# algbio/founderblockgraphs

Hardware: AMD Instinct MI355X
Metric: MSA columns segmented/sec (higher is better)
Workload: dtype u32

## Files before the change

### founderblockgraphs_amd/csrc/fbg_internal.h

```cpp
#pragma once
#include <cstring>
#include <cstdlib>
#include <hip/hip_runtime.h>
#include <stdint.h>
#include <string>
#include "../../include/fbg_hip.h"

#define FBG_WAVE 64

struct DevBuf {
    void *p = nullptr;
    size_t cap = 0;
    template <class T> T *as() const { return reinterpret_cast<T *>(p); }
};

struct Stager {
    void *base = nullptr;
    size_t slot_bytes = 0;
    int nslots = 0;
    hipEvent_t *ev = nullptr;
    hipStream_t stream = nullptr;
};

struct StageTimer {
// ... 72 lines not shown
    DevBuf gbits;
    DevBuf gwin_rows;
    const uint64_t *grs_ebits = nullptr;
    bool grs_flagged = false;
    bool pairs_similar = false;
    bool grs_ties_done = false;
    bool gpart = false;
    bool grs_part_failed = false;
    uint32_t grs_t = 1;
    uint64_t grs_redone = 0;
    bool spanned = false;
    DevBuf sp_cells;
    DevBuf sp_flagT;
    bool sp_key_flags = false;
    uint64_t alloc_calls = 0, alloc_us = 0;
    int sp_decline = 0;
    bool sp_key_flags_sorted = false;
    DevBuf sp_cwin;
    DevBuf sp_tiles, sp_gstart, sp_gcol, sp_gflags, sp_rstart, sp_rid, sp_gplo, sp_gphi, sp_gval, sp_odd, sp_irr, sp_chain, sp_slow, sp_mins;
    uint32_t sp_chain_n = 0, sp_slow_n = 0;
    uint64_t sp_G = 0, sp_R = 0, sp_n_irr = 0, sp_work = 0;
    uint32_t sp_n_odd[4] = {0, 0, 0, 0}, sp_odd_cap = 0;
    const uint32_t *sort_payload = nullptr;
    int64_t msd_decline = -1;
    int dp_kind = -1;
    bool cells_built = false;
    uint8_t ignore_tab[256] = {0};
    uint64_t *rk_keys = nullptr;
    int rk_b = 0, rk_key_bits = 0, rk_K = 0;
    int rk_layout = 0, rk_pb = 0;
    bool part_active = false;
    int part = 0, nparts = 1;
    uint64_t part_count = 0;
    uint64_t part_T = 0;
    uint32_t part_gmin = 0;

    DevBuf keysA, keysB, valsA, valsB, grp, flags, list, tie_list, big_groups, tmp, small, scalars;
    DevBuf msd_ext;
    DevBuf kargs;
    alignas(16) unsigned char kargs_host[512];
    DevBuf msd_w, msd_v;
    DevBuf dp_a, dp_b, dp_c, dp_d, dp_e, dp_f, dp_g, dp_h, io_a, io_b, io_c, io_d;
    DevBuf bt_up, bt_dep;
    DevBuf ps_a, ps_b, ps_c, ps_d, ps_e, ps_f, ps_g, ps_h;

    StageTimer timers[FBG_STAGE_COUNT];
};

int fbg_fail(fbg_ctx *ctx, int code, const char *fmt, ...);
#define FBG_HIP_TRY(ctx, expr)                                                              \
    do {                                                                                    \
        hipError_t e_ = (expr);                                                             \
        if (e_ != hipSuccess)                                                               \
            return fbg_fail((ctx), e_ == hipErrorOutOfMemory ? FBG_ERR_OOM : FBG_ERR_HIP,   \
                            "%s failed: %s (%s:%d)", #expr, hipGetErrorString(e_), __FILE__, \
                            __LINE__);                                                      \
    } while (0)
#define FBG_TRY(expr)                \
    do {                             \
        int rc_ = (expr);            \
        if (rc_ != FBG_OK) return rc_; \
    } while (0)

int fbg_reserve(fbg_ctx *ctx, DevBuf &b, size_t bytes);
int fbg_upload(fbg_ctx *ctx, void *d_dst, const void *h_src, size_t bytes);
int fbg_download(fbg_ctx *ctx, void *h_dst, const void *d_src, size_t bytes);
void fbg_release(fbg_ctx *ctx, DevBuf &b);
// ... 77 lines not shown
```

### founderblockgraphs_amd/csrc/rank_common.h

```cpp
#pragma once
#include "fbg_internal.h"
#include "text_cmp.h"

#define RS_TG 4

__device__ __forceinline__ uint32_t rs_key_lcp(uint64_t a, uint64_t c, int b, int key_bits)
{
    const uint64_t d = a ^ c;
    const uint32_t bits = (uint32_t)(__clzll((long long)d) - (64 - key_bits));
    const uint32_t inv_b = (65536u + (uint32_t)b - 1) / (uint32_t)b;
    return (bits * inv_b) >> 16;
}

struct RankArgs {
    uint32_t magic32;
    uint64_t magic64;
    uint64_t *keys;
    uint32_t *vals;
    uint64_t pmask;
    int pb;
    const uint8_t *T;
    uint64_t N, n;
    uint64_t Ntext;
    uint64_t own_lo, own_hi;
    int first_part, last_part;
    int part_mode;
    int values_only;
    uint32_t row_len;
    uint32_t g_min;
    int b, key_bits, K, reversed;
    uint32_t *gmax;
    uint32_t *cand;
    uint32_t *blk_count;
    uint32_t region;
    uint32_t *ties;
    uint32_t *tie_count;
    uint32_t tie_region;
    uint2 *pairs;
    int pair_codes;
    unsigned long long *pair_stats;
    uint32_t *pair_count;
    uint32_t *pm;
    uint32_t *big;
    unsigned long long *counters;
};

struct Slot {
    uint64_t key;
    uint64_t pos;
    uint32_t col;
    uint32_t rem;
};

__device__ __forceinline__ uint32_t rs_col_of_rem(const RankArgs &a, uint32_t rem)
{
    return rem == 0 ? (uint32_t)a.n : (a.reversed ? rem - 1 : (uint32_t)a.n - rem);
}
template <int L> struct PosT { typedef uint32_t type; };
template <> struct PosT<FBG_SLOTS_WIDE> { typedef uint64_t type; };
template <int L> __device__ __forceinline__ uint64_t rs_key(const RankArgs &a, uint64_t k) { return a.keys[k] >> a.pb; }
template <int L> __device__ __forceinline__ uint64_t rs_pos_of(const RankArgs &a, uint64_t w, uint32_t v)
{
    if (L == FBG_SLOTS_PACKED) return w & a.pmask;
    if (L == FBG_SLOTS_WIDE) return ((w & a.pmask) << 32) | v;
    return v;
}
template <int L> __device__ __forceinline__ uint64_t rs_pos(const RankArgs &a, uint64_t k)
{
    return rs_pos_of<L>(a, L == FBG_SLOTS_PAIRS ? 0ull : a.keys[k], L == FBG_SLOTS_PACKED ? 0u : a.vals[k]);
}
template <int L> __device__ __forceinline__ void rs_set_pos(const RankArgs &a, uint64_t k, uint64_t p)
{
    if (L == FBG_SLOTS_PACKED) a.keys[k] = (a.keys[k] & ~a.pmask) | p;
    else if (L == FBG_SLOTS_WIDE) { a.keys[k] = (a.keys[k] & ~a.pmask) | (p >> 32); a.vals[k] = (uint32_t)p; }
    else a.vals[k] = (uint32_t)p;
// ... 139 lines not shown
        uint32_t mr = 0;
        for (;;) {
            const uint32_t rj = v.rem(j);
            mr = max(mr, rj);
            run = run || rj == rem;
            cnt++;
            if (j + 1 >= hi_i || v.key(j + 1) != kn) break;
            if (cnt == RS_TG) { run = true; break; }
            j++;
        }
        mrn = mr;
    }
    if (edge || run) { want_cand = true; return; }
    const uint32_t lp = has_prev ? min(min(rs_key_lcp(kp, key, a.b, a.key_bits), rem), mrp) : 0u;
    const uint32_t ln = has_next ? min(min(rs_key_lcp(key, kn, a.b, a.key_bits), rem), mrn) : 0u;
    const uint32_t g = max(lp, ln) + 1;
    if (g >= a.g_min || rem <= 64) rs_update(a, rs_col_of_rem(a, rem), g);
}


static inline int rs_layout(const KeyGeom &g) { return g.packed ? FBG_SLOTS_PACKED : g.wide ? FBG_SLOTS_WIDE : FBG_SLOTS_PAIRS; }

static inline void rs_args_init(fbg_ctx *ctx, RankArgs &a, uint64_t *keys, uint32_t *vals, uint64_t slots, int layout, int pb, int b,
                         int key_bits, int K)
{
    a.keys = keys; a.vals = vals; a.T = ctx->text.as<uint8_t>();
    a.pb = layout != FBG_SLOTS_PAIRS ? pb : 0; a.pmask = layout != FBG_SLOTS_PAIRS ? (1ull << pb) - 1 : 0;
    a.N = slots; a.Ntext = ctx->N; a.n = ctx->n; a.row_len = (uint32_t)(ctx->n + 1);
    a.own_lo = 0; a.own_hi = slots; a.first_part = a.last_part = 1; a.part_mode = 0; a.values_only = 0;
    a.magic32 = (uint32_t)((1ull << 32) / (ctx->n + 1));
    a.magic64 = ~0ull / (ctx->n + 1);
    a.b = b; a.key_bits = key_bits; a.K = K; a.reversed = ctx->reversed;
    a.gmax = ctx->gmax.as<uint32_t>();
    a.cand = nullptr; a.pm = nullptr; a.blk_count = nullptr; a.region = 0;
    a.ties = nullptr; a.tie_count = nullptr; a.tie_region = 0; a.pairs = nullptr; a.pair_count = nullptr; a.pair_codes = 0;
    a.pair_stats = nullptr;
    a.big = ctx->big_groups.as<uint32_t>();
    a.counters = ctx->scalars.as<unsigned long long>() + 32;
    a.g_min = 0;
}

static inline void rs_remember(fbg_ctx *ctx, uint64_t *keys, uint32_t *vals, const KeyGeom &g)
{
    ctx->rk_keys = keys; ctx->sa_ptr = vals;
    ctx->rk_layout = rs_layout(g); ctx->rk_pb = g.pb;
    ctx->rk_b = g.b; ctx->rk_key_bits = g.key_bits; ctx->rk_K = g.K;
}
```

### founderblockgraphs_amd/csrc/rank_scan.hip

```cpp
#include <algorithm>
#include <cstring>
#include <vector>
#include "fbg_internal.h"
#include "text_cmp.h"
#include <rocprim/rocprim.hpp>

#include "rank_common.h"

#define RS_ITEMS 4
#define RS_THREADS 256
#define RS_CHUNK (RS_THREADS * RS_ITEMS)

template <int L, bool PLAIN> __global__ __launch_bounds__(RS_THREADS) __attribute__((amdgpu_waves_per_eu(7, 8))) void k_rank_scan(RankArgs a)
{
    __shared__ uint64_t skey[RS_CHUNK + 2 * RS_HALO];
    __shared__ uint32_t srem[RS_CHUNK + 2 * RS_HALO];
    __shared__ uint16_t sq[RS_CHUNK];
    __shared__ uint32_t sqn, s_cand_n, s_tie_n;
    const int lane = threadIdx.x & 63;
    const uint64_t nchunks = (a.own_hi - a.own_lo + RS_CHUNK - 1) / RS_CHUNK;
    if (threadIdx.x == 0) { s_cand_n = 0; s_tie_n = 0; }
    uint64_t w[RS_ITEMS + 1];
    uint32_t v[RS_ITEMS + 1];
    const int my_i = RS_HALO + RS_ITEMS * (int)threadIdx.x;
    const int halo_i = (int)threadIdx.x < RS_HALO ? (int)threadIdx.x : RS_CHUNK + (int)threadIdx.x;
    auto fetch = [&](uint64_t c) {
        const uint64_t base = a.own_lo + c * RS_CHUNK;
        const int lo_i = c == 0 ? RS_HALO : 0;
        const int hi_i = (int)min((uint64_t)(RS_CHUNK + 2 * RS_HALO), a.own_hi - base + RS_HALO);
#pragma unroll
        for (int r = 0; r < RS_ITEMS; r++) {
            w[r] = 0; v[r] = 0;
            if (my_i + r < hi_i) {
                w[r] = a.keys[base + (uint64_t)(my_i + r - RS_HALO)];
                if (L != FBG_SLOTS_PACKED) v[r] = a.vals[base + (uint64_t)(my_i + r - RS_HALO)];
            }
        }
        w[RS_ITEMS] = 0; v[RS_ITEMS] = 0;
// ... 407 lines not shown
            const uint32_t ln = k + 1 < N ? rs_key_lcp(key, kn, b, key_bits) : 0u;
            bin = min(max(lp, ln) + 1, 63u);
        }
    }
    {
        const int lane = threadIdx.x & 63;
        unsigned long long rest = __ballot(bin != 0xffffffffu);
        while (rest) {
            const int l = __ffsll((long long)rest) - 1;
            const uint32_t v = __shfl(bin, l, 64);
            const unsigned long long same = __ballot(bin == v);
            if (lane == l) { if (v == 64) atomicAdd(&sties, (uint32_t)__popcll(same)); else atomicAdd(&sh[v], (uint32_t)__popcll(same)); }
            rest &= ~same;
        }
    }
    __syncthreads();
    if (threadIdx.x < 64 && sh[threadIdx.x]) atomicAdd(&hist[threadIdx.x], sh[threadIdx.x]);
    if (threadIdx.x == 0) {
        atomicAdd(&counters[2], (unsigned long long)sties);
        atomicAdd(&counters[3], (unsigned long long)min((uint64_t)256, N - (uint64_t)blockIdx.x * 1024 * 256));
    }
}

__global__ void k_count_unfilled(const uint32_t *__restrict__ gmax, uint64_t n, uint32_t g_min, int reversed,
                                 unsigned long long *__restrict__ counters)
{
    const uint64_t x = (uint64_t)blockIdx.x * blockDim.x + threadIdx.x;
    const uint64_t rem = reversed ? x + 1 : n - x;
    const bool miss = x < n && rem > 64 && gmax[x] < g_min;
    const unsigned long long mask = __ballot(miss);
    if ((threadIdx.x & 63) == 0 && mask) atomicAdd(&counters[1 + 3], (unsigned long long)__popcll(mask));
}

__global__ void k_cand_compact(const uint32_t *__restrict__ regions, const uint32_t *__restrict__ counts,
                               const uint32_t *__restrict__ offsets, uint32_t region, uint32_t *__restrict__ out)
{
    const uint32_t c = counts[blockIdx.x] < region ? counts[blockIdx.x] : region, o = offsets[blockIdx.x];
    for (uint32_t i = threadIdx.x; i < c; i += blockDim.x) out[o + i] = regions[(size_t)blockIdx.x * region + i];
}

#define RS_BIG_GROUPS 1024
#define RS_BIG_MEMBERS 8192
template <int L> __global__ void k_tie_groups(RankArgs a, uint64_t T, int by_list)
{
    const uint64_t t = (uint64_t)blockIdx.x * blockDim.x + threadIdx.x;
    if (t >= T) return;
    const uint64_t k0 = by_list ? (uint64_t)a.cand[t] : a.own_lo + t;
    const uint64_t key = rs_key<L>(a, k0);
    if (k0 > a.own_lo && rs_key<L>(a, k0 - 1) == key) return;
    if (k0 + 1 >= a.own_hi || rs_key<L>(a, k0 + 1) != key) return;
    uint32_t s = 1;
    while (k0 + s < a.own_hi && s <= RS_BIG_MEMBERS && rs_key<L>(a, k0 + s) == key) s++;
    if (s > 64) {
        if (s > RS_BIG_MEMBERS) { a.counters[1] = 1; return; }
        const unsigned long long e = atomicAdd(&a.counters[5], 1ull);
        if (e >= RS_BIG_GROUPS) { a.counters[1] = 1; return; }
        a.big[2 * e] = (uint32_t)k0;
        a.big[2 * e + 1] = s;
        return;
    }
    typedef typename PosT<L>::type pos_t;
    pos_t pos[64];
    uint32_t from = (uint32_t)a.K;
    for (uint32_t i = 0; i < s; i++) {
        pos[i] = (pos_t)rs_pos<L>(a, k0 + i);
        if (rs_rem<L>(a, pos[i]) < (uint32_t)a.K) from = 0;
    }
    for (uint32_t i = 1; i < s; i++) {
        const pos_t cur = pos[i];
        uint32_t j = i;
        while (j > 0) {
            const pos_t o = pos[j - 1];
            const uint32_t h = fbg_extend_match(a.T, (uint64_t)o + from, (uint64_t)cur + from, 0);
            if (a.T[(uint64_t)o + from + h] < a.T[(uint64_t)cur + from + h]) break;
            pos[j] = o;
            j--;
        }
        pos[j] = cur;
    }
    for (uint32_t i = 0; i < s; i++) rs_set_pos<L>(a, k0 + i, pos[i]);
}

template <int L> __global__ __launch_bounds__(256) void k_tie_big(RankArgs a, int exact)
{
    __shared__ uint32_t pos_lo[RS_BIG_MEMBERS];
    __shared__ uint8_t pos_hi[L == FBG_SLOTS_WIDE ? RS_BIG_MEMBERS : 1];
    __shared__ uint8_t cls[RS_BIG_MEMBERS];
    __shared__ uint32_t offs[66];
    __shared__ uint32_t q_start, q_count;
    if (blockIdx.x >= a.counters[5]) return;
    const uint64_t k0 = a.big[2 * blockIdx.x];
    const uint32_t s = a.big[2 * blockIdx.x + 1];
    auto member = [&](uint32_t i) -> uint64_t {
        return L == FBG_SLOTS_WIDE ? ((uint64_t)pos_hi[L == FBG_SLOTS_WIDE ? i : 0] << 32) | pos_lo[i] : (uint64_t)pos_lo[i];
    };
    if (threadIdx.x < 66) offs[threadIdx.x] = 0;
    __syncthreads();
    for (uint32_t i = threadIdx.x; i < s; i += blockDim.x) {
        const uint64_t p = rs_pos<L>(a, k0 + i);
        const uint32_t c = min(rs_rem<L>(a, p), (uint32_t)a.K);
        pos_lo[i] = (uint32_t)p;
        if (L == FBG_SLOTS_WIDE) pos_hi[L == FBG_SLOTS_WIDE ? i : 0] = (uint8_t)(p >> 32);
        cls[i] = (uint8_t)c;
        atomicAdd(&offs[c + 1], 1u);
    }
    __syncthreads();
    if (threadIdx.x == 0) {
        q_count = offs[a.K + 1];
        for (int c = 1; c <= a.K + 1; c++) offs[c] += offs[c - 1];
        q_start = offs[a.K];
    }
    __syncthreads();
    if (!exact) {
// ... 25 lines not shown
    for (uint32_t i = threadIdx.x; i < s; i += blockDim.x) {
        const uint64_t p = member(i);
        uint32_t rank = 0;
        for (uint32_t j = 0; j < s; j++) {
            if (j == i) continue;
            const uint64_t o = member(j);
            const uint32_t h = fbg_extend_match(a.T, o, p, 0);
            rank += a.T[o + h] < a.T[p + h] ? 1u : 0u;
        }
        rs_set_pos<L>(a, k0 + rank, p);
    }
}

template <int L> __device__ __forceinline__ uint32_t rs_slot_lcp(const RankArgs &a, uint64_t k)
{
    if (k == (a.first_part ? a.own_lo : 0) || k >= (a.last_part ? a.own_hi : a.N)) return 0;
    const Slot x = rs_slot<L>(a, k - 1), y = rs_slot<L>(a, k);
    if (x.key != y.key) return min(min(rs_key_lcp(x.key, y.key, a.b, a.key_bits), x.rem), y.rem);
    const uint32_t from = (x.rem < (uint32_t)a.K || y.rem < (uint32_t)a.K) ? 0u : (uint32_t)a.K;
    return fbg_clamp_lcp(fbg_extend_match(a.T, (uint64_t)x.pos + from, (uint64_t)y.pos + from, 0) + from);
}

template <int L> __global__ void k_rank_materialize(RankArgs a, uint32_t *sa, uint32_t *isa, uint32_t *pl, uint32_t *pr)
{
    const uint64_t k = (uint64_t)blockIdx.x * blockDim.x + threadIdx.x;
    if (k >= a.N) return;
    const uint32_t p = (uint32_t)rs_pos<L>(a, k);
    sa[k] = p;
    isa[p] = (uint32_t)k;
    pl[p] = rs_slot_lcp<L>(a, k);
    pr[p] = rs_slot_lcp<L>(a, k + 1);
}

template <int L> __global__ void k_runs(RankArgs a, uint64_t T)
{
    const uint64_t t = (uint64_t)blockIdx.x * blockDim.x + threadIdx.x;
    if (t >= T) return;
    const uint64_t k0 = a.cand[t];
    const uint32_t col = rs_col<L>(a, k0);
    if (col == a.n) return;
    if (k0 > a.own_lo && rs_col<L>(a, k0 - 1) == col) return;
    const uint64_t lo_slot = a.first_part ? a.own_lo : 0, hi_slot = a.last_part ? a.own_hi : a.N;
    uint64_t ks = k0;
    while (ks > lo_slot && rs_col<L>(a, ks - 1) == col) ks--;
    if (ks == 0 && !a.first_part) { a.counters[1] = 1; return; }
    uint32_t run = rs_slot_lcp<L>(a, ks);
    uint64_t s = ks;
    for (;;) {
        if (s >= k0 && s < a.own_hi) a.pm[t + (s - k0)] = run;
        if (s + 1 >= hi_slot || rs_col<L>(a, s + 1) != col) break;
        s++;
        run = min(run, rs_slot_lcp<L>(a, s));
    }
    if (s + 1 == a.N && !a.last_part) { a.counters[1] = 1; return; }
    uint32_t rmin = 0xffffffffu;
    for (;; s--) {
        rmin = min(rmin, rs_slot_lcp<L>(a, s + 1));
        if (s >= k0 && s < a.own_hi) rs_update(a, col, max(a.pm[t + (s - k0)], rmin) + 1);
        if (s == ks || s <= k0) break;
    }
}

struct FinishArgs {
    const uint32_t *gmax;
    uint64_t n, x0, x1;
    int mode, disable_tricks;
    uint64_t *out;
};

__global__ void k_rank_finish(FinishArgs a)
{
    const uint64_t x = a.x0 + (uint64_t)blockIdx.x * blockDim.x + threadIdx.x;
    if (x >= a.x1) return;
    const unsigned long long g = a.gmax[x];
    if (a.mode == FBG_SCAN_V) {
        a.out[x] = g <= x + 1 ? x + 1 - g : x + 1;
        return;
    }
    unsigned long long fx = x;
    const bool any_active = a.disable_tricks || x != 0;
    if (any_active && g > 0) {
        const unsigned long long gg = x + g;
        const unsigned long long fi = gg > a.n ? (a.disable_tricks ? a.n : a.n - 1) : gg - 1;
        fx = max(fx, fi);
    }
    a.out[x] = max((unsigned long long)a.out[x], fx);
}

template <class F> static int rs_with_tmp(fbg_ctx *ctx, F &&call)
{
    size_t bytes = 0;
    hipError_t e = call(nullptr, bytes);
    if (e != hipSuccess) return fbg_fail(ctx, FBG_ERR_HIP, "rocprim size query: %s", hipGetErrorString(e));
    FBG_TRY(fbg_reserve(ctx, ctx->tmp, bytes));
    size_t have = ctx->tmp.cap;
    e = call(ctx->tmp.p, have);
    if (e != hipSuccess) return fbg_fail(ctx, FBG_ERR_HIP, "rocprim call: %s", hipGetErrorString(e));
    return FBG_OK;
}

#define RS_LAUNCH(kernel, layout, grid, block, st, ...)                                                     \
    do {                                                                                                    \
        if ((layout) == FBG_SLOTS_PACKED) hipLaunchKernelGGL((kernel<FBG_SLOTS_PACKED>), grid, block, 0, st, __VA_ARGS__);  \
        else if ((layout) == FBG_SLOTS_WIDE) hipLaunchKernelGGL((kernel<FBG_SLOTS_WIDE>), grid, block, 0, st, __VA_ARGS__); \
        else hipLaunchKernelGGL((kernel<FBG_SLOTS_PAIRS>), grid, block, 0, st, __VA_ARGS__);                                \
    } while (0)

#define RS_LAUNCH_SCAN(layout, plain, grid, st, args)                                                                         \
    do {                                                                                                                     \
        const dim3 blk_(RS_THREADS);                                                                                         \
        if ((layout) == FBG_SLOTS_PACKED) { if (plain) hipLaunchKernelGGL((k_rank_scan<FBG_SLOTS_PACKED, true>), grid, blk_, 0, st, args);   \
                                            else hipLaunchKernelGGL((k_rank_scan<FBG_SLOTS_PACKED, false>), grid, blk_, 0, st, args); }      \
        else if ((layout) == FBG_SLOTS_WIDE) { if (plain) hipLaunchKernelGGL((k_rank_scan<FBG_SLOTS_WIDE, true>), grid, blk_, 0, st, args);  \
                                               else hipLaunchKernelGGL((k_rank_scan<FBG_SLOTS_WIDE, false>), grid, blk_, 0, st, args); }     \
        else { if (plain) hipLaunchKernelGGL((k_rank_scan<FBG_SLOTS_PAIRS, true>), grid, blk_, 0, st, args);                               \
               else hipLaunchKernelGGL((k_rank_scan<FBG_SLOTS_PAIRS, false>), grid, blk_, 0, st, args); }                                  \
    } while (0)

static int rs_fork(fbg_ctx *ctx)
{
    if (!ctx->aux) {
        FBG_HIP_TRY(ctx, hipStreamCreateWithFlags(&ctx->aux, hipStreamNonBlocking));
        FBG_HIP_TRY(ctx, hipEventCreateWithFlags(&ctx->aux_fork, hipEventDisableTiming));
        FBG_HIP_TRY(ctx, hipEventCreateWithFlags(&ctx->aux_join, hipEventDisableTiming));
    }
    FBG_HIP_TRY(ctx, hipEventRecord(ctx->aux_fork, ctx->stream));
    FBG_HIP_TRY(ctx, hipStreamWaitEvent(ctx->aux, ctx->aux_fork, 0));
    ctx->aux_pending = true;
    return FBG_OK;
}
static int rs_join(fbg_ctx *ctx)
{
    if (!ctx->aux_pending) return FBG_OK;
    ctx->aux_pending = false;
    FBG_HIP_TRY(ctx, hipEventRecord(ctx->aux_join, ctx->aux));
    FBG_HIP_TRY(ctx, hipStreamWaitEvent(ctx->stream, ctx->aux_join, 0));
    return FBG_OK;
}

static int rs_order_candidates(fbg_ctx *ctx, RankArgs &a, int layout, uint64_t T, int *launches)
{
    hipStream_t st = ctx->stream;
    FBG_TRY(fbg_reserve(ctx, ctx->dp_a, T * 4));
    FBG_TRY(fbg_reserve(ctx, ctx->dp_b, T * 4));
    uint32_t *sorted = ctx->dp_a.as<uint32_t>();
    uint32_t *flat = ctx->dp_e.as<uint32_t>();
    FBG_TRY(rs_with_tmp(ctx, [&](void *tmp, size_t &bytes) {
        return rocprim::radix_sort_keys(tmp, bytes, flat, sorted, (size_t)T, 0u, 32u, st);
    }));
    a.cand = sorted;
    a.pm = ctx->dp_b.as<uint32_t>();
    RS_LAUNCH(k_tie_groups, layout, dim3(fbg_blocks(T, 64)), dim3(64), st, a, T, 1);
    RS_LAUNCH(k_tie_big, layout, dim3(RS_BIG_GROUPS), dim3(256), st, a, 0);
    *launches += 3;
    return FBG_OK;
}

static int rs_classify(fbg_ctx *ctx, RankArgs &a, int layout, uint64_t *T_out, int *launches)
{
    hipStream_t st = ctx->stream;
    const uint64_t own = a.own_hi - a.own_lo;
    const unsigned rs_blocks = fbg_blocks(own, RS_CHUNK, 256 * 16);
    const uint32_t region = (uint32_t)((own / rs_blocks) / 8 + 256);
    const uint32_t tie_region = (uint32_t)((own / rs_blocks) / 6 + 256);
    FBG_TRY(fbg_reserve(ctx, ctx->list, (size_t)rs_blocks * region * 4));
    FBG_TRY(fbg_reserve(ctx, ctx->tie_list, (size_t)rs_blocks * tie_region * 4));
    FBG_TRY(fbg_reserve(ctx, ctx->big_groups, RS_BIG_GROUPS * 8));
    a.big = ctx->big_groups.as<uint32_t>();
    FBG_TRY(fbg_reserve(ctx, ctx->dp_c, (size_t)(rs_blocks + 1) * 4));
    FBG_TRY(fbg_reserve(ctx, ctx->dp_d, (size_t)(rs_blocks + 1) * 4));
    FBG_TRY(fbg_reserve(ctx, ctx->dp_f, (size_t)(rs_blocks + 1) * 4));
    FBG_HIP_TRY(ctx, hipMemsetAsync(ctx->dp_c.p, 0, (size_t)(rs_blocks + 1) * 4, st));
    FBG_HIP_TRY(ctx, hipMemsetAsync(ctx->dp_f.p, 0, (size_t)(rs_blocks + 1) * 4, st));
    a.cand = ctx->list.as<uint32_t>();
    a.blk_count = ctx->dp_c.as<uint32_t>(); a.region = region;
    a.ties = ctx->tie_list.as<uint32_t>();
    a.tie_count = ctx->dp_f.as<uint32_t>(); a.tie_region = tie_region;
    FBG_TRY(fbg_stage_begin(ctx, FBG_STAGE_RANK_KERNEL));
    LeanArgs lf;
    const bool lean = layout == FBG_SLOTS_PACKED && a.g_min > (uint32_t)a.K && !a.values_only && !a.part_mode && !ctx->opt.rank_no_lean &&
                      rs_lean_setup(a, a.pb, rs_blocks, &lf);
    ctx->rank_lean_launched = lean ? 1 : 0;
    if (lean)
    {
        if (ctx->msd_ext_valid && a.keys == ctx->keysA.as<uint64_t>() && a.b == 2 && a.pb <= 30 && a.own_lo == 0 && a.own_hi == ctx->N) {
            lf.ext = ctx->msd_ext.as<uint8_t>();
            a.pair_codes = 1;
        }
        a.pair_stats = ctx->scalars.as<unsigned long long>() + 112;
        FBG_HIP_TRY(ctx, hipMemsetAsync(a.pair_stats, 0, 2 * sizeof(unsigned long long), st));
        FBG_TRY(fbg_reserve(ctx, ctx->ps_g, (size_t)rs_blocks * tie_region * 8));
        FBG_TRY(fbg_reserve(ctx, ctx->ps_h, (size_t)rs_blocks * 4));
        a.pairs = ctx->ps_g.as<uint2>(); a.pair_count = ctx->ps_h.as<uint32_t>();
        static_assert(sizeof(RankArgs) <= sizeof(ctx->kargs_host), "room for the scan's arguments");
        FBG_TRY(fbg_reserve(ctx, ctx->kargs, sizeof(RankArgs)));
        memcpy(ctx->kargs_host, &a, sizeof(RankArgs));
        FBG_HIP_TRY(ctx, hipMemcpyAsync(ctx->kargs.p, ctx->kargs_host, sizeof(RankArgs), hipMemcpyHostToDevice, st));
        hipLaunchKernelGGL(k_rank_scan_lean, dim3(rs_blocks), dim3(RL_THREADS), 0, st, (const RankArgs *)ctx->kargs.p, lf);
    }
    else
        RS_LAUNCH_SCAN(layout, a.g_min <= (uint32_t)a.K || a.values_only, dim3(rs_blocks), st, a);
    FBG_TRY(fbg_stage_end(ctx, FBG_STAGE_RANK_KERNEL, 1));
    {
        hipStream_t ts = st;
        if (!ctx->opt.no_aux_stream) { FBG_TRY(rs_fork(ctx)); ts = ctx->aux; }
        if (lean) hipLaunchKernelGGL(k_tie_pairs, dim3(rs_blocks), dim3(256), 0, ts, a);
        RS_LAUNCH(k_tie_simple, layout, dim3(rs_blocks), dim3(256), ts, a);
    }
    *launches += 2;
    const int rc_rest = [&]() -> int {
        uint32_t *d_counts = a.blk_count, *d_offs = ctx->dp_d.as<uint32_t>();
        FBG_TRY(rs_with_tmp(ctx, [&](void *tmp, size_t &bytes) {
            return rocprim::exclusive_scan(tmp, bytes, d_counts, d_offs, 0u, (size_t)(rs_blocks + 1), rocprim::plus<uint32_t>(), st);
        }));
        uint32_t *d_max = reinterpret_cast<uint32_t *>(a.counters + 6);
        FBG_TRY(rs_with_tmp(ctx, [&](void *tmp, size_t &bytes) {
            return rocprim::reduce(tmp, bytes, d_counts, d_max, 0u, (size_t)rs_blocks, rocprim::maximum<uint32_t>(), st);
        }));
        uint32_t tot = 0, mx = 0;
        FBG_HIP_TRY(ctx, hipMemcpyAsync(&tot, d_offs + rs_blocks, 4, hipMemcpyDeviceToHost, st));
        FBG_HIP_TRY(ctx, hipMemcpyAsync(&mx, d_max, 4, hipMemcpyDeviceToHost, st));
        FBG_HIP_TRY(ctx, hipStreamSynchronize(st));
        const uint64_t T = tot;
        *T_out = T;
        if (mx > region) { *T_out = ~0ull; return rs_join(ctx); }
        if (T > 0) {
            FBG_TRY(fbg_reserve(ctx, ctx->dp_e, T * 4));
            uint32_t *flat = ctx->dp_e.as<uint32_t>();
            hipLaunchKernelGGL(k_cand_compact, dim3(rs_blocks), dim3(256), 0, st, a.cand, d_counts, d_offs, region, flat);
            FBG_TRY(rs_order_candidates(ctx, a, layout, T, launches));
        }
        return FBG_OK;
    }();
    if (rc_rest != FBG_OK) { (void)rs_join(ctx); return rc_rest; }
    return FBG_OK;
}

static int rs_pick_threshold(fbg_ctx *ctx, RankArgs &a, const uint64_t *keys, uint64_t count, const KeyGeom &geom, int *reject,
                             int *launches)
{
    *reject = 0;
    if (count <= (1u << 22)) return FBG_OK;
    hipStream_t st = ctx->stream;
    unsigned long long *cnt = a.counters;
    unsigned int *d_hist = reinterpret_cast<unsigned int *>(cnt + 8);
    FBG_HIP_TRY(ctx, hipMemsetAsync(d_hist, 0, 64 * sizeof(unsigned int), st));
    hipLaunchKernelGGL(k_tie_sample, dim3(fbg_blocks(count, 1024 * 256)), dim3(256), 0, st, keys, a.pb, count, geom.b, geom.key_bits,
                       cnt, d_hist);
    (*launches)++;
    unsigned long long hs[4];
    unsigned int hh[64];
    FBG_HIP_TRY(ctx, hipMemcpyAsync(hs, cnt, sizeof(hs), hipMemcpyDeviceToHost, st));
    FBG_HIP_TRY(ctx, hipMemcpyAsync(hh, d_hist, sizeof(hh), hipMemcpyDeviceToHost, st));
    FBG_HIP_TRY(ctx, hipStreamSynchronize(st));
    if (hs[2] * 4 > hs[3]) { *reject = 1; return FBG_OK; }
    if (!ctx->opt.rank_no_threshold) {
        const double need = 32.0 / (double)ctx->m * (double)hs[3];
        unsigned long long above = 0;
        for (int g = 63; g >= 1; g--) {
            above += hh[g];
            if ((double)above >= need) { a.g_min = (uint32_t)g; break; }
        }
        if ((double)hs[2] / (double)hs[3] * (double)ctx->m >= 32.0) a.g_min = (uint32_t)geom.K + 1;
    }
    return FBG_OK;
}

int fbg_rank_scan_try(fbg_ctx *ctx, uint64_t *keys, uint32_t *vals, const KeyGeom &geom, int *done)
{
    *done = 0;
    ctx->ranked = false;
    ctx->part_active = false;
    ctx->ext_pairs = ctx->text_pairs = -1;
    ctx->rank_lean_used = ctx->rank_lean_launched = 0;
    const uint64_t N = ctx->N, n = ctx->n;
    const int layout = rs_layout(geom);
    hipStream_t st = ctx->stream;
    FBG_TRY(fbg_stage_begin(ctx, FBG_STAGE_RANKSCAN));
    unsigned long long *cnt = ctx->scalars.as<unsigned long long>() + 32;
    int launches = 0;
    FBG_TRY(fbg_reserve(ctx, ctx->gmax, (n + 1) * 4));
    RankArgs a;
    rs_args_init(ctx, a, keys, vals, N, layout, geom.pb, geom.b, geom.key_bits, geom.K);
    uint64_t T = 0;
    FBG_HIP_TRY(ctx, hipMemsetAsync(cnt, 0, 8 * sizeof(unsigned long long), st));
    FBG_HIP_TRY(ctx, hipMemsetAsync(ctx->gmax.p, 0, (n + 1) * 4, st));
    int reject = 0;
    FBG_TRY(rs_pick_threshold(ctx, a, keys, N, geom, &reject, &launches));
    if (reject) return fbg_stage_end(ctx, FBG_STAGE_RANKSCAN, launches);
    FBG_TRY(rs_classify(ctx, a, layout, &T, &launches));
    if (T == ~0ull) return fbg_stage_end(ctx, FBG_STAGE_RANKSCAN, launches);
    if (T > 0) {
        RS_LAUNCH(k_runs, layout, dim3(fbg_blocks(T, 64)), dim3(64), st, a, T);
        launches++;
    }
    FBG_TRY(rs_join(ctx));
    unsigned long long h[5], ps[2] = {0, 0};
    if (a.g_min > 1)
        hipLaunchKernelGGL(k_count_unfilled, dim3(fbg_blocks(n, 256)), dim3(256), 0, st, a.gmax, n, a.g_min, a.reversed, cnt);
    FBG_HIP_TRY(ctx, hipMemcpyAsync(h, cnt, sizeof(h), hipMemcpyDeviceToHost, st));
    if (a.pair_stats) FBG_HIP_TRY(ctx, hipMemcpyAsync(ps, a.pair_stats, sizeof(ps), hipMemcpyDeviceToHost, st));
    FBG_HIP_TRY(ctx, hipStreamSynchronize(st));
    ctx->ext_pairs = (int64_t)ps[0];
    ctx->text_pairs = (int64_t)ps[1];
    launches++;
    if (h[1] != 0) return fbg_stage_end(ctx, FBG_STAGE_RANKSCAN, launches);
    if (a.g_min > 1 && h[4] != 0) {
        a.g_min = 0;
        a.values_only = 1;
        RS_LAUNCH_SCAN(layout, true, dim3(fbg_blocks(N, RS_CHUNK, 256 * 16)), st, a);
        launches++;
    }
    FBG_HIP_TRY(ctx, hipGetLastError());
    ctx->n_exc = 0;
    ctx->ranked = true;
    ctx->rank_lean_used = ctx->rank_lean_launched;
    rs_remember(ctx, keys, vals, geom);
    *done = 1;
    return fbg_stage_end(ctx, FBG_STAGE_RANKSCAN, launches);
}

__global__ void k_halo_export(const uint64_t *__restrict__ keys, const uint32_t *__restrict__ vals, uint64_t own_lo,
                              uint64_t own_hi, uint64_t ok, uint8_t *__restrict__ blob)
{
    uint64_t *bk = reinterpret_cast<uint64_t *>(blob);
    uint32_t *bv = reinterpret_cast<uint32_t *>(blob + 2 * FBG_PART_HALO * 8);
    uint64_t *tail = reinterpret_cast<uint64_t *>(blob + 2 * FBG_PART_HALO * 12);
    const uint32_t t = threadIdx.x;
// ... 8 lines not shown
                              uint64_t *__restrict__ keys, uint32_t *__restrict__ vals)
{
    const uint32_t t = threadIdx.x;
    if (part > 0) {
        const uint8_t *bl = blobs + (size_t)(part - 1) * FBG_PART_HALO_BYTES;
        keys[t] = reinterpret_cast<const uint64_t *>(bl)[FBG_PART_HALO + t];
        if (vals) vals[t] = reinterpret_cast<const uint32_t *>(bl + 2 * FBG_PART_HALO * 8)[FBG_PART_HALO + t];
    }
    if (part + 1 < nparts) {
        const uint8_t *bl = blobs + (size_t)(part + 1) * FBG_PART_HALO_BYTES;
        keys[own_hi + t] = reinterpret_cast<const uint64_t *>(bl)[t];
        if (vals) vals[own_hi + t] = reinterpret_cast<const uint32_t *>(bl + 2 * FBG_PART_HALO * 8)[t];
    }
}

static void rs_part_args(fbg_ctx *ctx, RankArgs &a)
{
    rs_args_init(ctx, a, ctx->rk_keys, ctx->sa_ptr, ctx->part_count + 2 * FBG_PART_HALO, ctx->rk_layout, ctx->rk_pb, ctx->rk_b,
                 ctx->rk_key_bits, ctx->rk_K);
    a.own_lo = FBG_PART_HALO; a.own_hi = FBG_PART_HALO + ctx->part_count;
    a.first_part = ctx->part == 0; a.last_part = ctx->part + 1 == ctx->nparts;
    a.part_mode = ctx->nparts > 1;
}

int fbg_rank_part_classify(fbg_ctx *ctx, uint64_t *keys, uint32_t *vals, uint64_t count, const KeyGeom &geom, int pre_ok,
                           uint8_t *d_blob, int *ok)
{
    const uint64_t n = ctx->n;
    hipStream_t st = ctx->stream;
    FBG_TRY(fbg_stage_begin(ctx, FBG_STAGE_RANKSCAN));
    int launches = 0;
    ctx->ranked = false;
    ctx->part_count = count;
    ctx->part_T = 0;
    rs_remember(ctx, keys, vals, geom);
    const int layout = rs_layout(geom);
    FBG_TRY(fbg_reserve(ctx, ctx->gmax, (n + 1) * 4));
    unsigned long long *cnt = ctx->scalars.as<unsigned long long>() + 32;
    FBG_HIP_TRY(ctx, hipMemsetAsync(cnt, 0, 8 * sizeof(unsigned long long), st));
    FBG_HIP_TRY(ctx, hipMemsetAsync(ctx->gmax.p, 0, (n + 1) * 4, st));
    int good = pre_ok && count >= 2 * FBG_PART_HALO;
    RankArgs a;
    rs_part_args(ctx, a);
    if (good) {
        int reject = 0;
        FBG_TRY(rs_pick_threshold(ctx, a, keys + a.own_lo, count, geom, &reject, &launches));
        if (reject) good = 0;
    }
    ctx->part_gmin = a.g_min;
    if (good) {
        uint64_t T = 0;
        FBG_TRY(rs_classify(ctx, a, layout, &T, &launches));
        FBG_TRY(rs_join(ctx));
        if (T == ~0ull) good = 0;
        else {
            ctx->part_T = T;
            unsigned long long h[2];
            FBG_HIP_TRY(ctx, hipMemcpyAsync(h, cnt, sizeof(h), hipMemcpyDeviceToHost, st));
            FBG_HIP_TRY(ctx, hipStreamSynchronize(st));
            if (h[1] != 0) good = 0;
        }
    }
    hipLaunchKernelGGL(k_halo_export, dim3(1), dim3(2 * FBG_PART_HALO), 0, st, keys, vals, a.own_lo, a.own_hi,
                       (uint64_t)good | ((uint64_t)a.g_min << 8), d_blob);
    launches++;
    FBG_HIP_TRY(ctx, hipGetLastError());
    *ok = good;
    return fbg_stage_end(ctx, FBG_STAGE_RANKSCAN, launches);
}

int fbg_rank_part_runs(fbg_ctx *ctx, const uint8_t *d_blobs, uint32_t *d_gmax, int *ok)
{
    const uint64_t n = ctx->n;
    hipStream_t st = ctx->stream;
    FBG_TRY(fbg_stage_begin(ctx, FBG_STAGE_RANKSCAN));
    int launches = 0;
    std::vector<uint8_t> hb((size_t)ctx->nparts * FBG_PART_HALO_BYTES);
    FBG_HIP_TRY(ctx, hipMemcpyAsync(hb.data(), d_blobs, hb.size(), hipMemcpyDeviceToHost, st));
    FBG_HIP_TRY(ctx, hipStreamSynchronize(st));
    int good = 1;
    uint32_t gmin_all = 0;
    for (int p = 0; p < ctx->nparts; p++) {
        uint64_t tail[2];
        memcpy(tail, hb.data() + (size_t)p * FBG_PART_HALO_BYTES + 2 * FBG_PART_HALO * 12, sizeof(tail));
        if (!(tail[0] & 1)) good = 0;
        gmin_all = std::max(gmin_all, (uint32_t)(tail[0] >> 8));
    }
    ctx->part_gmin = gmin_all;
    if (good) {
        RankArgs a;
        rs_part_args(ctx, a);
        a.cand = ctx->dp_a.as<uint32_t>(); a.pm = ctx->dp_b.as<uint32_t>();
        hipLaunchKernelGGL(k_halo_import, dim3(1), dim3(FBG_PART_HALO), 0, st, d_blobs, ctx->part, ctx->nparts, a.own_lo,
                           a.own_hi, a.keys, a.vals);
        launches++;
        if (ctx->part_T > 0) {
            RS_LAUNCH(k_runs, ctx->rk_layout, dim3(fbg_blocks(ctx->part_T, 64)), dim3(64), st, a, ctx->part_T);
            launches++;
            unsigned long long h[2];
            FBG_HIP_TRY(ctx, hipMemcpyAsync(h, a.counters, sizeof(h), hipMemcpyDeviceToHost, st));
            FBG_HIP_TRY(ctx, hipStreamSynchronize(st));
            if (h[1] != 0) good = 0;
        }
    }
    FBG_HIP_TRY(ctx, hipMemcpyAsync(d_gmax, ctx->gmax.p, (n + 1) * 4, hipMemcpyDeviceToDevice, st));
    const uint32_t verdict = good ? 0u : 1u;
    FBG_HIP_TRY(ctx, hipMemcpyAsync(d_gmax + n, &verdict, 4, hipMemcpyHostToDevice, st));
    FBG_HIP_TRY(ctx, hipStreamSynchronize(st));
    *ok = good;
    return fbg_stage_end(ctx, FBG_STAGE_RANKSCAN, launches);
}

int fbg_rank_part_unfilled(fbg_ctx *ctx, uint64_t *unfilled)
{
    *unfilled = 0;
    if (ctx->part_gmin <= 1) return FBG_OK;
    hipStream_t st = ctx->stream;
    unsigned long long *cnt = ctx->scalars.as<unsigned long long>() + 32;
    FBG_HIP_TRY(ctx, hipMemsetAsync(cnt + 4, 0, sizeof(unsigned long long), st));
    hipLaunchKernelGGL(k_count_unfilled, dim3(fbg_blocks(ctx->n, 256)), dim3(256), 0, st, ctx->gmax.as<uint32_t>(), ctx->n, ctx->part_gmin,
                       ctx->reversed, cnt);
    unsigned long long h = 0;
    FBG_HIP_TRY(ctx, hipMemcpyAsync(&h, cnt + 4, sizeof(h), hipMemcpyDeviceToHost, st));
    FBG_HIP_TRY(ctx, hipStreamSynchronize(st));
    *unfilled = h;
    return FBG_OK;
}

int fbg_rank_part_rescan(fbg_ctx *ctx)
{
    FBG_TRY(fbg_stage_begin(ctx, FBG_STAGE_RANKSCAN));
    RankArgs a;
    rs_part_args(ctx, a);
    a.g_min = 0;
    a.values_only = 1;
    RS_LAUNCH_SCAN(ctx->rk_layout, true, dim3(fbg_blocks(ctx->part_count, RS_CHUNK, 256 * 16)), ctx->stream, a);
    FBG_HIP_TRY(ctx, hipGetLastError());
    ctx->part_gmin = 0;
    return fbg_stage_end(ctx, FBG_STAGE_RANKSCAN, 1);
}

int fbg_rank_finish(fbg_ctx *ctx, uint64_t x0, uint64_t x1, int mode, int disable_tricks, uint64_t *d_out)
{
    FinishArgs f;
    f.gmax = ctx->gmax.as<uint32_t>();
    f.n = ctx->n; f.x0 = x0; f.x1 = x1; f.mode = mode; f.disable_tricks = disable_tricks; f.out = d_out;
    hipLaunchKernelGGL(k_rank_finish, dim3(fbg_blocks(x1 - x0, 256)), dim3(256), 0, ctx->stream, f);
    FBG_HIP_TRY(ctx, hipGetLastError());
    return FBG_OK;
}

int fbg_rank_materialize(fbg_ctx *ctx, uint32_t *d_sa, uint32_t *d_isa, uint32_t *d_pl, uint32_t *d_pr)
{
    RankArgs a;
    rs_args_init(ctx, a, ctx->rk_keys, ctx->sa_ptr, ctx->N, ctx->rk_layout, ctx->rk_pb, ctx->rk_b, ctx->rk_key_bits, ctx->rk_K);
    FBG_TRY(fbg_reserve(ctx, ctx->big_groups, RS_BIG_GROUPS * 8));
    a.big = ctx->big_groups.as<uint32_t>();
    FBG_HIP_TRY(ctx, hipMemsetAsync(a.counters + 5, 0, sizeof(unsigned long long), ctx->stream));
    RS_LAUNCH(k_tie_groups, ctx->rk_layout, dim3(fbg_blocks(ctx->N, 256)), dim3(256), ctx->stream, a, ctx->N, 0);
    RS_LAUNCH(k_tie_big, ctx->rk_layout, dim3(RS_BIG_GROUPS), dim3(256), ctx->stream, a, 1);
    RS_LAUNCH(k_rank_materialize, ctx->rk_layout, dim3(fbg_blocks(ctx->N, 256)), dim3(256), ctx->stream, a, d_sa, d_isa, d_pl, d_pr);
    FBG_HIP_TRY(ctx, hipGetLastError());
    return FBG_OK;
}
```

Measured before the change: 59.78 million.

## Process rank-scan candidates per block in place, dropping global compaction and sort

Candidate slots are now processed directly from their per-block regions by new k_tie_classes and k_runs kernels, which replace the rocprim exclusive scan, max reduce, compaction, radix sort and the host readback and sync that sized them. Tie groups are resolved one wave at a time with ballots and shuffles, and k_runs updates each run-boundary slot independently instead of walking the whole run with a scratch array. This removes several launches and a host round-trip on the critical path. In exchange, correctness relies on unsorted candidates and a per-slot boundary formulation, and region overflow is now detected inside the kernels.

After: 59.07 million, median of 2. About the same (-1.2%).

```diff
diff --git a/founderblockgraphs_amd/csrc/fbg_internal.h b/founderblockgraphs_amd/csrc/fbg_internal.h
--- a/founderblockgraphs_amd/csrc/fbg_internal.h
+++ b/founderblockgraphs_amd/csrc/fbg_internal.h
@@ -128,7 +128,8 @@
     bool part_active = false;
     int part = 0, nparts = 1;
     uint64_t part_count = 0;
-    uint64_t part_T = 0;
+    unsigned part_blocks = 0;
+    uint32_t part_region = 0;
     uint32_t part_gmin = 0;
 
     DevBuf keysA, keysB, valsA, valsB, grp, flags, list, tie_list, big_groups, tmp, small, scalars;
diff --git a/founderblockgraphs_amd/csrc/rank_common.h b/founderblockgraphs_amd/csrc/rank_common.h
--- a/founderblockgraphs_amd/csrc/rank_common.h
+++ b/founderblockgraphs_amd/csrc/rank_common.h
@@ -40,7 +40,6 @@
     int pair_codes;
     unsigned long long *pair_stats;
     uint32_t *pair_count;
-    uint32_t *pm;
     uint32_t *big;
     unsigned long long *counters;
 };
@@ -246,7 +245,7 @@
     a.magic64 = ~0ull / (ctx->n + 1);
     a.b = b; a.key_bits = key_bits; a.K = K; a.reversed = ctx->reversed;
     a.gmax = ctx->gmax.as<uint32_t>();
-    a.cand = nullptr; a.pm = nullptr; a.blk_count = nullptr; a.region = 0;
+    a.cand = nullptr; a.blk_count = nullptr; a.region = 0;
     a.ties = nullptr; a.tie_count = nullptr; a.tie_region = 0; a.pairs = nullptr; a.pair_count = nullptr; a.pair_codes = 0;
     a.pair_stats = nullptr;
     a.big = ctx->big_groups.as<uint32_t>();
diff --git a/founderblockgraphs_amd/csrc/rank_scan.hip b/founderblockgraphs_amd/csrc/rank_scan.hip
--- a/founderblockgraphs_amd/csrc/rank_scan.hip
+++ b/founderblockgraphs_amd/csrc/rank_scan.hip
@@ -3,7 +3,6 @@
 #include <vector>
 #include "fbg_internal.h"
 #include "text_cmp.h"
-#include <rocprim/rocprim.hpp>
 
 #include "rank_common.h"
 
@@ -477,33 +476,31 @@
     if ((threadIdx.x & 63) == 0 && mask) atomicAdd(&counters[1 + 3], (unsigned long long)__popcll(mask));
 }
 
-__global__ void k_cand_compact(const uint32_t *__restrict__ regions, const uint32_t *__restrict__ counts,
-                               const uint32_t *__restrict__ offsets, uint32_t region, uint32_t *__restrict__ out)
-{
-    const uint32_t c = counts[blockIdx.x] < region ? counts[blockIdx.x] : region, o = offsets[blockIdx.x];
-    for (uint32_t i = threadIdx.x; i < c; i += blockDim.x) out[o + i] = regions[(size_t)blockIdx.x * region + i];
-}
-
 #define RS_BIG_GROUPS 1024
 #define RS_BIG_MEMBERS 8192
-template <int L> __global__ void k_tie_groups(RankArgs a, uint64_t T, int by_list)
+template <int L> __device__ uint32_t rs_big_group(const RankArgs &a, uint64_t k0, uint64_t key, uint32_t s)
+{
+    while (k0 + s < a.own_hi && s <= RS_BIG_MEMBERS && rs_key<L>(a, k0 + s) == key) s++;
+    if (s > 64) {
+        if (s > RS_BIG_MEMBERS) { a.counters[1] = 1; return s; }
+        const unsigned long long e = atomicAdd(&a.counters[5], 1ull);
+        if (e >= RS_BIG_GROUPS) { a.counters[1] = 1; return s; }
+        a.big[2 * e] = (uint32_t)k0;
+        a.big[2 * e + 1] = s;
+    }
+    return s;
+}
+
+template <int L> __global__ void k_tie_groups(RankArgs a, uint64_t T)
 {
     const uint64_t t = (uint64_t)blockIdx.x * blockDim.x + threadIdx.x;
     if (t >= T) return;
-    const uint64_t k0 = by_list ? (uint64_t)a.cand[t] : a.own_lo + t;
+    const uint64_t k0 = a.own_lo + t;
     const uint64_t key = rs_key<L>(a, k0);
     if (k0 > a.own_lo && rs_key<L>(a, k0 - 1) == key) return;
     if (k0 + 1 >= a.own_hi || rs_key<L>(a, k0 + 1) != key) return;
-    uint32_t s = 1;
-    while (k0 + s < a.own_hi && s <= RS_BIG_MEMBERS && rs_key<L>(a, k0 + s) == key) s++;
-    if (s > 64) {
-        if (s > RS_BIG_MEMBERS) { a.counters[1] = 1; return; }
-        const unsigned long long e = atomicAdd(&a.counters[5], 1ull);
-        if (e >= RS_BIG_GROUPS) { a.counters[1] = 1; return; }
-        a.big[2 * e] = (uint32_t)k0;
-        a.big[2 * e + 1] = s;
-        return;
-    }
+    const uint32_t s = rs_big_group<L>(a, k0, key, 1);
+    if (s > 64) return;
     typedef typename PosT<L>::type pos_t;
     pos_t pos[64];
     uint32_t from = (uint32_t)a.K;
@@ -524,6 +521,65 @@
         pos[j] = cur;
     }
     for (uint32_t i = 0; i < s; i++) rs_set_pos<L>(a, k0 + i, pos[i]);
+}
+
+__device__ __forceinline__ uint64_t rs_shfl64(uint64_t v, int src)
+{
+    return ((uint64_t)(uint32_t)__shfl((int)(uint32_t)(v >> 32), src, 64) << 32) | (uint32_t)__shfl((int)(uint32_t)v, src, 64);
+}
+
+template <int L> __global__ __launch_bounds__(256) void k_tie_classes(RankArgs a)
+{
+    const uint32_t have = a.blk_count[blockIdx.x];
+    if (have > a.region) { if (threadIdx.x == 0) a.counters[1] = 1; return; }
+    const int lane = threadIdx.x & 63;
+    const uint32_t K = (uint32_t)a.K;
+    for (uint32_t e0 = threadIdx.x & ~63u; e0 < have; e0 += blockDim.x) {
+        uint64_t k = 0;
+        bool head = false;
+        if (e0 + lane < have) {
+            k = a.cand[(size_t)blockIdx.x * a.region + e0 + lane];
+            const uint64_t key = rs_key<L>(a, k);
+            head = !(k > a.own_lo && rs_key<L>(a, k - 1) == key) && k + 1 < a.own_hi && rs_key<L>(a, k + 1) == key;
+        }
+        for (unsigned long long heads = __ballot(head); heads; heads &= heads - 1) {
+            const int hl = __ffsll((long long)heads) - 1;
+            const uint64_t k0 = rs_shfl64(k, hl);
+            const uint64_t key = rs_key<L>(a, k0);
+            const uint64_t slot = k0 + (uint64_t)lane;
+            const bool same = slot < a.own_hi && rs_key<L>(a, slot) == key;
+            const unsigned long long sm = __ballot(same);
+            const uint32_t s = ~sm ? (uint32_t)(__ffsll((long long)~sm) - 1) : 64u;
+            if (s == 64) {
+                uint32_t big = 0;
+                if (lane == 0) big = rs_big_group<L>(a, k0, key, 64) > 64 ? 1u : 0u;
+                if (__shfl((int)big, 0, 64)) continue;
+            }
+            const bool in = (uint32_t)lane < s;
+            const uint64_t pos = in ? rs_pos<L>(a, slot) : 0ull;
+            const uint32_t rem = in ? rs_rem<L>(a, pos) : 0u;
+            const uint32_t rem0 = (uint32_t)__shfl((int)rem, 0, 64);
+            if (!__ballot(in && rem != rem0)) continue;
+            const uint32_t cls = min(rem, K);
+            uint32_t d = 0;
+            for (uint32_t j = 0; j < s; j++) {
+                const uint32_t cj = (uint32_t)__shfl((int)cls, (int)j, 64);
+                d += (cj < cls || (cj == cls && cls < K && j < (uint32_t)lane)) ? 1u : 0u;
+            }
+            const unsigned long long full = __ballot(in && cls == K);
+            if (__popcll(full) > 1) {
+                for (unsigned long long rest = full; rest; rest &= rest - 1) {
+                    const int j = __ffsll((long long)rest) - 1;
+                    const uint64_t o = rs_shfl64(pos, j);
+                    if (((full >> lane) & 1ull) && j != lane) {
+                        const uint32_t h = fbg_extend_match(a.T, o + K, pos + K, 0);
+                        d += a.T[o + K + h] < a.T[pos + K + h] ? 1u : 0u;
+                    }
+                }
+            }
+            if (in) rs_set_pos<L>(a, k0 + d, pos);
+        }
+    }
 }
 
 template <int L> __global__ __launch_bounds__(256) void k_tie_big(RankArgs a, int exact)
@@ -615,32 +671,22 @@
     pr[p] = rs_slot_lcp<L>(a, k + 1);
 }
 
-template <int L> __global__ void k_runs(RankArgs a, uint64_t T)
-{
-    const uint64_t t = (uint64_t)blockIdx.x * blockDim.x + threadIdx.x;
-    if (t >= T) return;
-    const uint64_t k0 = a.cand[t];
-    const uint32_t col = rs_col<L>(a, k0);
-    if (col == a.n) return;
-    if (k0 > a.own_lo && rs_col<L>(a, k0 - 1) == col) return;
+template <int L> __global__ __launch_bounds__(256) void k_runs(RankArgs a)
+{
+    const uint32_t have = a.blk_count[blockIdx.x];
+    if (have > a.region) { if (threadIdx.x == 0) a.counters[1] = 1; return; }
     const uint64_t lo_slot = a.first_part ? a.own_lo : 0, hi_slot = a.last_part ? a.own_hi : a.N;
-    uint64_t ks = k0;
-    while (ks > lo_slot && rs_col<L>(a, ks - 1) == col) ks--;
-    if (ks == 0 && !a.first_part) { a.counters[1] = 1; return; }
-    uint32_t run = rs_slot_lcp<L>(a, ks);
-    uint64_t s = ks;
-    for (;;) {
-        if (s >= k0 && s < a.own_hi) a.pm[t + (s - k0)] = run;
-        if (s + 1 >= hi_slot || rs_col<L>(a, s + 1) != col) break;
-        s++;
-        run = min(run, rs_slot_lcp<L>(a, s));
-    }
-    if (s + 1 == a.N && !a.last_part) { a.counters[1] = 1; return; }
-    uint32_t rmin = 0xffffffffu;
-    for (;; s--) {
-        rmin = min(rmin, rs_slot_lcp<L>(a, s + 1));
-        if (s >= k0 && s < a.own_hi) rs_update(a, col, max(a.pm[t + (s - k0)], rmin) + 1);
-        if (s == ks || s <= k0) break;
+    for (uint32_t e = threadIdx.x; e < have; e += blockDim.x) {
+        const uint64_t k = a.cand[(size_t)blockIdx.x * a.region + e];
+        const uint32_t col = rs_col<L>(a, k);
+        if (col == a.n) continue;
+        const bool left = k == lo_slot || rs_col<L>(a, k - 1) != col;
+        const bool right = k + 1 >= hi_slot || rs_col<L>(a, k + 1) != col;
+        if (!left && !right) continue;
+        uint32_t g = 0;
+        if (left) g = rs_slot_lcp<L>(a, k);
+        if (right) g = max(g, rs_slot_lcp<L>(a, k + 1));
+        rs_update(a, col, g + 1);
     }
 }
 
@@ -668,18 +714,6 @@
         fx = max(fx, fi);
     }
     a.out[x] = max((unsigned long long)a.out[x], fx);
-}
-
-template <class F> static int rs_with_tmp(fbg_ctx *ctx, F &&call)
-{
-    size_t bytes = 0;
-    hipError_t e = call(nullptr, bytes);
-    if (e != hipSuccess) return fbg_fail(ctx, FBG_ERR_HIP, "rocprim size query: %s", hipGetErrorString(e));
-    FBG_TRY(fbg_reserve(ctx, ctx->tmp, bytes));
-    size_t have = ctx->tmp.cap;
-    e = call(ctx->tmp.p, have);
-    if (e != hipSuccess) return fbg_fail(ctx, FBG_ERR_HIP, "rocprim call: %s", hipGetErrorString(e));
-    return FBG_OK;
 }
 
 #define RS_LAUNCH(kernel, layout, grid, block, st, ...)                                                     \
@@ -721,25 +755,7 @@
     return FBG_OK;
 }
 
-static int rs_order_candidates(fbg_ctx *ctx, RankArgs &a, int layout, uint64_t T, int *launches)
-{
-    hipStream_t st = ctx->stream;
-    FBG_TRY(fbg_reserve(ctx, ctx->dp_a, T * 4));
-    FBG_TRY(fbg_reserve(ctx, ctx->dp_b, T * 4));
-    uint32_t *sorted = ctx->dp_a.as<uint32_t>();
-    uint32_t *flat = ctx->dp_e.as<uint32_t>();
-    FBG_TRY(rs_with_tmp(ctx, [&](void *tmp, size_t &bytes) {
-        return rocprim::radix_sort_keys(tmp, bytes, flat, sorted, (size_t)T, 0u, 32u, st);
-    }));
-    a.cand = sorted;
-    a.pm = ctx->dp_b.as<uint32_t>();
-    RS_LAUNCH(k_tie_groups, layout, dim3(fbg_blocks(T, 64)), dim3(64), st, a, T, 1);
-    RS_LAUNCH(k_tie_big, layout, dim3(RS_BIG_GROUPS), dim3(256), st, a, 0);
-    *launches += 3;
-    return FBG_OK;
-}
-
-static int rs_classify(fbg_ctx *ctx, RankArgs &a, int layout, uint64_t *T_out, int *launches)
+static int rs_classify(fbg_ctx *ctx, RankArgs &a, int layout, unsigned *blocks, int *launches)
 {
     hipStream_t st = ctx->stream;
     const uint64_t own = a.own_hi - a.own_lo;
@@ -750,11 +766,10 @@
     FBG_TRY(fbg_reserve(ctx, ctx->tie_list, (size_t)rs_blocks * tie_region * 4));
     FBG_TRY(fbg_reserve(ctx, ctx->big_groups, RS_BIG_GROUPS * 8));
     a.big = ctx->big_groups.as<uint32_t>();
-    FBG_TRY(fbg_reserve(ctx, ctx->dp_c, (size_t)(rs_blocks + 1) * 4));
-    FBG_TRY(fbg_reserve(ctx, ctx->dp_d, (size_t)(rs_blocks + 1) * 4));
-    FBG_TRY(fbg_reserve(ctx, ctx->dp_f, (size_t)(rs_blocks + 1) * 4));
-    FBG_HIP_TRY(ctx, hipMemsetAsync(ctx->dp_c.p, 0, (size_t)(rs_blocks + 1) * 4, st));
-    FBG_HIP_TRY(ctx, hipMemsetAsync(ctx->dp_f.p, 0, (size_t)(rs_blocks + 1) * 4, st));
+    FBG_TRY(fbg_reserve(ctx, ctx->dp_c, (size_t)rs_blocks * 4));
+    FBG_TRY(fbg_reserve(ctx, ctx->dp_f, (size_t)rs_blocks * 4));
+    FBG_HIP_TRY(ctx, hipMemsetAsync(ctx->dp_c.p, 0, (size_t)rs_blocks * 4, st));
+    FBG_HIP_TRY(ctx, hipMemsetAsync(ctx->dp_f.p, 0, (size_t)rs_blocks * 4, st));
     a.cand = ctx->list.as<uint32_t>();
     a.blk_count = ctx->dp_c.as<uint32_t>(); a.region = region;
     a.ties = ctx->tie_list.as<uint32_t>();
@@ -790,32 +805,10 @@
         if (lean) hipLaunchKernelGGL(k_tie_pairs, dim3(rs_blocks), dim3(256), 0, ts, a);
         RS_LAUNCH(k_tie_simple, layout, dim3(rs_blocks), dim3(256), ts, a);
     }
-    *launches += 2;
-    const int rc_rest = [&]() -> int {
-        uint32_t *d_counts = a.blk_count, *d_offs = ctx->dp_d.as<uint32_t>();
-        FBG_TRY(rs_with_tmp(ctx, [&](void *tmp, size_t &bytes) {
-            return rocprim::exclusive_scan(tmp, bytes, d_counts, d_offs, 0u, (size_t)(rs_blocks + 1), rocprim::plus<uint32_t>(), st);
-        }));
-        uint32_t *d_max = reinterpret_cast<uint32_t *>(a.counters + 6);
-        FBG_TRY(rs_with_tmp(ctx, [&](void *tmp, size_t &bytes) {
-            return rocprim::reduce(tmp, bytes, d_counts, d_max, 0u, (size_t)rs_blocks, rocprim::maximum<uint32_t>(), st);
-        }));
-        uint32_t tot = 0, mx = 0;
-        FBG_HIP_TRY(ctx, hipMemcpyAsync(&tot, d_offs + rs_blocks, 4, hipMemcpyDeviceToHost, st));
-        FBG_HIP_TRY(ctx, hipMemcpyAsync(&mx, d_max, 4, hipMemcpyDeviceToHost, st));
-        FBG_HIP_TRY(ctx, hipStreamSynchronize(st));
-        const uint64_t T = tot;
-        *T_out = T;
-        if (mx > region) { *T_out = ~0ull; return rs_join(ctx); }
-        if (T > 0) {
-            FBG_TRY(fbg_reserve(ctx, ctx->dp_e, T * 4));
-            uint32_t *flat = ctx->dp_e.as<uint32_t>();
-            hipLaunchKernelGGL(k_cand_compact, dim3(rs_blocks), dim3(256), 0, st, a.cand, d_counts, d_offs, region, flat);
-            FBG_TRY(rs_order_candidates(ctx, a, layout, T, launches));
-        }
-        return FBG_OK;
-    }();
-    if (rc_rest != FBG_OK) { (void)rs_join(ctx); return rc_rest; }
+    RS_LAUNCH(k_tie_classes, layout, dim3(rs_blocks), dim3(256), st, a);
+    RS_LAUNCH(k_tie_big, layout, dim3(RS_BIG_GROUPS), dim3(256), st, a, 0);
+    *launches += 4;
+    *blocks = rs_blocks;
     return FBG_OK;
 }
 
@@ -865,18 +858,15 @@
     FBG_TRY(fbg_reserve(ctx, ctx->gmax, (n + 1) * 4));
     RankArgs a;
     rs_args_init(ctx, a, keys, vals, N, layout, geom.pb, geom.b, geom.key_bits, geom.K);
-    uint64_t T = 0;
     FBG_HIP_TRY(ctx, hipMemsetAsync(cnt, 0, 8 * sizeof(unsigned long long), st));
     FBG_HIP_TRY(ctx, hipMemsetAsync(ctx->gmax.p, 0, (n + 1) * 4, st));
     int reject = 0;
     FBG_TRY(rs_pick_threshold(ctx, a, keys, N, geom, &reject, &launches));
     if (reject) return fbg_stage_end(ctx, FBG_STAGE_RANKSCAN, launches);
-    FBG_TRY(rs_classify(ctx, a, layout, &T, &launches));
-    if (T == ~0ull) return fbg_stage_end(ctx, FBG_STAGE_RANKSCAN, launches);
-    if (T > 0) {
-        RS_LAUNCH(k_runs, layout, dim3(fbg_blocks(T, 64)), dim3(64), st, a, T);
-        launches++;
-    }
+    unsigned blocks = 0;
+    FBG_TRY(rs_classify(ctx, a, layout, &blocks, &launches));
+    RS_LAUNCH(k_runs, layout, dim3(blocks), dim3(256), st, a);
+    launches++;
     FBG_TRY(rs_join(ctx));
     unsigned long long h[5], ps[2] = {0, 0};
     if (a.g_min > 1)
@@ -951,7 +941,7 @@
     int launches = 0;
     ctx->ranked = false;
     ctx->part_count = count;
-    ctx->part_T = 0;
+    ctx->part_blocks = 0;
     rs_remember(ctx, keys, vals, geom);
     const int layout = rs_layout(geom);
     FBG_TRY(fbg_reserve(ctx, ctx->gmax, (n + 1) * 4));
@@ -968,17 +958,15 @@
     }
     ctx->part_gmin = a.g_min;
     if (good) {
-        uint64_t T = 0;
-        FBG_TRY(rs_classify(ctx, a, layout, &T, &launches));
+        unsigned blocks = 0;
+        FBG_TRY(rs_classify(ctx, a, layout, &blocks, &launches));
         FBG_TRY(rs_join(ctx));
-        if (T == ~0ull) good = 0;
-        else {
-            ctx->part_T = T;
-            unsigned long long h[2];
-            FBG_HIP_TRY(ctx, hipMemcpyAsync(h, cnt, sizeof(h), hipMemcpyDeviceToHost, st));
-            FBG_HIP_TRY(ctx, hipStreamSynchronize(st));
-            if (h[1] != 0) good = 0;
-        }
+        ctx->part_blocks = blocks;
+        ctx->part_region = a.region;
+        unsigned long long h[2];
+        FBG_HIP_TRY(ctx, hipMemcpyAsync(h, cnt, sizeof(h), hipMemcpyDeviceToHost, st));
+        FBG_HIP_TRY(ctx, hipStreamSynchronize(st));
+        if (h[1] != 0) good = 0;
     }
     hipLaunchKernelGGL(k_halo_export, dim3(1), dim3(2 * FBG_PART_HALO), 0, st, keys, vals, a.own_lo, a.own_hi,
                        (uint64_t)good | ((uint64_t)a.g_min << 8), d_blob);
@@ -1009,17 +997,13 @@
     if (good) {
         RankArgs a;
         rs_part_args(ctx, a);
-        a.cand = ctx->dp_a.as<uint32_t>(); a.pm = ctx->dp_b.as<uint32_t>();
+        a.cand = ctx->list.as<uint32_t>(); a.blk_count = ctx->dp_c.as<uint32_t>(); a.region = ctx->part_region;
         hipLaunchKernelGGL(k_halo_import, dim3(1), dim3(FBG_PART_HALO), 0, st, d_blobs, ctx->part, ctx->nparts, a.own_lo,
                            a.own_hi, a.keys, a.vals);
         launches++;
-        if (ctx->part_T > 0) {
-            RS_LAUNCH(k_runs, ctx->rk_layout, dim3(fbg_blocks(ctx->part_T, 64)), dim3(64), st, a, ctx->part_T);
+        if (ctx->part_blocks > 0) {
+            RS_LAUNCH(k_runs, ctx->rk_layout, dim3(ctx->part_blocks), dim3(256), st, a);
             launches++;
-            unsigned long long h[2];
-            FBG_HIP_TRY(ctx, hipMemcpyAsync(h, a.counters, sizeof(h), hipMemcpyDeviceToHost, st));
-            FBG_HIP_TRY(ctx, hipStreamSynchronize(st));
-            if (h[1] != 0) good = 0;
         }
     }
     FBG_HIP_TRY(ctx, hipMemcpyAsync(d_gmax, ctx->gmax.p, (n + 1) * 4, hipMemcpyDeviceToDevice, st));
@@ -1076,7 +1060,7 @@
     FBG_TRY(fbg_reserve(ctx, ctx->big_groups, RS_BIG_GROUPS * 8));
     a.big = ctx->big_groups.as<uint32_t>();
     FBG_HIP_TRY(ctx, hipMemsetAsync(a.counters + 5, 0, sizeof(unsigned long long), ctx->stream));
-    RS_LAUNCH(k_tie_groups, ctx->rk_layout, dim3(fbg_blocks(ctx->N, 256)), dim3(256), ctx->stream, a, ctx->N, 0);
+    RS_LAUNCH(k_tie_groups, ctx->rk_layout, dim3(fbg_blocks(ctx->N, 256)), dim3(256), ctx->stream, a, ctx->N);
     RS_LAUNCH(k_tie_big, ctx->rk_layout, dim3(RS_BIG_GROUPS), dim3(256), ctx->stream, a, 1);
     RS_LAUNCH(k_rank_materialize, ctx->rk_layout, dim3(fbg_blocks(ctx->N, 256)), dim3(256), ctx->stream, a, d_sa, d_isa, d_pl, d_pr);
     FBG_HIP_TRY(ctx, hipGetLastError());
```
